# maxnorman569/Variational-Gridded-Gaussian-Processes

Hardware: NVIDIA B200
Metric: elbo_fwd_bwd_observations_per_sec (higher is better)
Workload: dtype f32

## Files before the change

### variational-gridded-gaussian-processes_b200/csrc/grid_b1.cuh

```cuda
#pragma once
#include "grid.cuh"

namespace vggp {

constexpr int FP_THREADS = 256;
constexpr int FP_WARPS = FP_THREADS / 32;
constexpr int FP_MAX_TASKS = 14;
constexpr int GEN_CHUNK = 32;
constexpr int GEN_THREADS = 256;
constexpr int FP_DET_BAND = 0;
constexpr int FP_DET_MALPHA = 3 * 512;
constexpr int FP_DET_TR = FP_DET_MALPHA + 1;
constexpr int FP_DET_LOGDET = FP_DET_TR + 8;
constexpr int FP_DET_SLOT = FP_DET_LOGDET + 8;

enum FpKind {
    FP_R = 0,
    FP_PROD,
    FP_ALPHA,
    FP_GA,
    FP_GAONLY,
    FP_DM,
    FP_DL,
    FP_QROW
};

struct FpTask {
    int kind, d, n, F;
    i64 inner, nfib;
    int tile0, ntiles;
    const double* s0;
    const double* s1;
    double* o0;
    const void* t0;
    void* t1;
    int direct;
    int pk;
};

struct FpPass {
    FpTask t[FP_MAX_TASKS];
    int ntasks;
    int D, obs_f32;
    i64 M;
    double ell_scale;
    const double* theta;
    double* gen[VGGP_MAX_D];
    double* acc[VGGP_MAX_D];
    double* sc;
    double* Qb[VGGP_MAX_D];
    void* bandT;
    int tab_off[VGGP_MAX_D];
    double* det;
    long long* dbg;
};

struct Mob { double a, b, c, d; };

__device__ __forceinline__ double pow2_inv_scale(double x) {
    const int e = (__double2hiint(x) >> 20) & 0x7ff;
    return __hiloint2double((2046 - e) << 20, 0);
}
__device__ __forceinline__ void mob_rescale(Mob& m) {
    const double sc = pow2_inv_scale(fmax(fmax(fabs(m.a), fabs(m.b)), fmax(fabs(m.c), fabs(m.d))));
    m.a *= sc; m.b *= sc; m.c *= sc; m.d *= sc;
}
__device__ __forceinline__ void mob_push(Mob& m, double p, double q) {
    const double na = fma(p, m.a, -q * m.c), nb = fma(p, m.b, -q * m.d);
    m.c = m.a; m.d = m.b; m.a = na; m.b = nb;
}

struct B1Coef { double a_in, a_bd, b; };
__device__ __forceinline__ B1Coef b1_coef(const GridDims& g, const double* theta, int d) {
    B1Coef c;
    const int n = g.n[d];
    c.a_bd = factor_entry(g, theta, d, 0, 0);
    c.a_in = factor_entry(g, theta, d, 1, 1);
    c.b = factor_entry(g, theta, d, 0, 1);
    if (n < 3) c.a_in = c.a_bd;
    return c;
}

template <typename T>
__global__ void __launch_bounds__(GEN_THREADS) k_b1_gens(const __grid_constant__ GridDims g, const double* __restrict__ theta,
                                                         double* __restrict__ acc_all, int acc_total,
                                                         double* __restrict__ theta_copy) {
    extern __shared__ double sm[];
    __shared__ double red[32];
    __shared__ double carry_d[GEN_THREADS], carry_e[GEN_THREADS];
    __shared__ Mob comp_d[GEN_THREADS / 2], comp_e[GEN_THREADS / 2];
    __shared__ int bad_flag;
    const int d = blockIdx.x;
    const int n = g.n[d];
    const int tid = threadIdx.x;
    auto G = [](int k) { return k + (k >> 5); };
    const int npad = n + (n >> 5) + 1;
    double* dd = sm;
    double* ee = dd + npad;
    double* rd = ee + npad;
    double* re = rd + npad;
    if (tid == 0) bad_flag = 0;
    if (d == 0) {
        if (tid < SC_COUNT) g.sc[tid] = 0.0;
        if (tid == 0) *g.info = 0;
        if (tid < 2 * g.D + 1) theta_copy[tid] = theta[tid];
    }
    for (int i = (int)blockIdx.x * GEN_THREADS + tid; i < acc_total; i += (int)gridDim.x * GEN_THREADS) acc_all[i] = 0.0;
    const B1Coef cf = b1_coef(g, theta, d);
    const double b2 = cf.b * cf.b;
    auto diag = [&](int k) { return (k == 0 || k == n - 1) ? cf.a_bd : cf.a_in; };
    const int nch = (n + GEN_CHUNK - 1) / GEN_CHUNK;
    const bool up = tid >= GEN_THREADS / 2;
    const int ch = up ? tid - GEN_THREADS / 2 : tid;
    if (ch < nch) {
        Mob m = {1.0, 0.0, 0.0, 1.0};
        const int k0 = ch * GEN_CHUNK, k1 = min(n, k0 + GEN_CHUNK);
        if (!up) {
            for (int k = max(k0, 1); k < k1; ++k) {
                mob_push(m, diag(k), b2);
                if ((k & 7) == 7) mob_rescale(m);
            }
            mob_rescale(m);
            comp_d[ch] = m;
        } else {
            for (int k = min(k1 - 1, n - 2); k >= k0; --k) {
                mob_push(m, diag(k), b2);
                if ((k & 7) == 0) mob_rescale(m);
            }
            mob_rescale(m);
            comp_e[ch] = m;
        }
    }
    __syncthreads();
    if (tid == 0) {
        double num = cf.a_bd, den = 1.0;
        for (int c = 0; c < nch; ++c) {
            carry_d[c] = num; carry_d[GEN_THREADS / 2 + c] = den;
            const Mob m = comp_d[c];
            const double nn = fma(m.a, num, m.b * den), dn = fma(m.c, num, m.d * den);
            const double sc = pow2_inv_scale(fmax(fabs(nn), fabs(dn)));
            num = nn * sc; den = dn * sc;
        }
    } else if (tid == 32) {
        double num = cf.a_bd, den = 1.0;
        for (int c = nch - 1; c >= 0; --c) {
            carry_e[c] = num; carry_e[GEN_THREADS / 2 + c] = den;
            const Mob m = comp_e[c];
            const double nn = fma(m.a, num, m.b * den), dn = fma(m.c, num, m.d * den);
            const double sc = pow2_inv_scale(fmax(fabs(nn), fabs(dn)));
            num = nn * sc; den = dn * sc;
        }
    }
    __syncthreads();
    if (ch < nch) {
        const int k0 = ch * GEN_CHUNK, k1 = min(n, k0 + GEN_CHUNK);
        bool bad = false;
        if (!up) {
            double prev = carry_d[ch] / carry_d[GEN_THREADS / 2 + ch];
            double r = 1.0 / prev;
            int k = k0;
            if (ch == 0) { dd[G(0)] = prev; rd[G(0)] = r; bad = !(prev > 0.0); k = 1; }
            for (; k < k1; ++k) {
                const double nxt = fma(-b2, r, diag(k));
                bad = bad || !(nxt > 0.0);
                double e = fma(-nxt, r, 1.0);
                double rn = fma(r, e, r);
                e = fma(-nxt, rn, 1.0);
                if (!(fabs(e) < 3e-16)) rn = 1.0 / nxt;
                r = rn;
                dd[G(k)] = nxt; rd[G(k)] = r;
            }
        } else {
            double nxt = carry_e[ch] / carry_e[GEN_THREADS / 2 + ch];
            double r = 1.0 / nxt;
            int k = k1 - 1;
            if (k1 == n) { ee[G(n - 1)] = nxt; re[G(n - 1)] = r; bad = !(nxt > 0.0); k = n - 2; }
            for (; k >= k0; --k) {
                const double cur = fma(-b2, r, diag(k));
                bad = bad || !(cur > 0.0);
                double e = fma(-cur, r, 1.0);
                double rn = fma(r, e, r);
                e = fma(-cur, rn, 1.0);
                if (!(fabs(e) < 3e-16)) rn = 1.0 / cur;
                r = rn;
                ee[G(k)] = cur; re[G(k)] = r;
            }
        }
        if (bad) bad_flag = 1;
    }
    __syncthreads();
    if (tid == 0 && bad_flag) atomicMax(g.info, d + 1);
    double* gen = g.gen[d];
    double prod = 1.0;
    double ld = 0.0;
    for (int i = tid; i < n; i += GEN_THREADS) {
        const double di = dd[G(i)];
        const double pdv = 1.0 / (di + ee[G(i)] - diag(i));
        const double ruv = (i + 1 < n) ? -cf.b * rd[G(i)] : 0.0;
        const double rlv = (i + 1 < n) ? -cf.b * re[G(i + 1)] : 0.0;
        gen[i] = pdv; gen[n + i] = ruv; gen[2 * n + i] = rlv;
        ee[G(i)] = pdv; dd[G(i)] = ruv;
        prod *= di;
        if (prod > 1e200 || prod < 1e-200) { ld += log(prod); prod = 1.0; }
    }
    ld += log(prod);
    __syncthreads();
    T* tab = reinterpret_cast<T*>(g.bandT) + g.tab_off[d];
    for (int i = tid; i < n; i += GEN_THREADS) {
        const bool last = (i + 1 >= n);
        const double A = ee[G(i)];
        const double B2 = last ? 0.0 : 2.0 * ee[G(i + 1)] * dd[G(i)];
        const double Cc = last ? 0.0 : ee[G(i + 1)];
        tab[i] = (T)A; tab[n + i] = (T)(B2 - 2.0 * A); tab[2 * n + i] = (T)(A - B2 + Cc);
    }
    ld = block_sum(ld, red);
    if (tid == 0) g.sc[SC_LOGDETK + d] = ld;
}

struct FpGeom {
    int n, S, pitch;
    unsigned magic;
};
__host__ __device__ inline FpGeom fp_geom(int n) {
    FpGeom q;
    q.n = n;
    q.S = (n + 31) / 32;
    int len = n + (n + q.S - 1) / q.S + 1;
    if (len < 32 * (q.S + 1) + 16) len = 32 * (q.S + 1) + 16;
    len = (len + 15) / 16 * 16 + 2;
    q.pitch = len;
    q.magic = (unsigned)((0x100000000ull + (unsigned long long)q.S - 1) / (unsigned long long)q.S);
    return q;
}
__host__ __device__ inline size_t fp_smem_bytes(int n, int F, bool aux) {
    const FpGeom q = fp_geom(n);
    const int narr = 1 + (aux ? 1 : 0) + (q.S > 16 ? 1 : 0);
    return sizeof(double) * ((size_t)5 * q.pitch + (size_t)narr * F * q.pitch);
}
__device__ __forceinline__ int fp_pidx(int i, unsigned SM) { return SM ? i + (int)__umulhi((unsigned)i, SM) : 2 * i; }

__host__ __device__ inline bool fp_kind_has_aux(int kind) { return kind == FP_GA || kind == FP_GAONLY || kind == FP_DL; }

__device__ __forceinline__ void fp_fibre(const FpGeom& q, const double* __restrict__ pd, const double* __restrict__ ru,
                                         const double* __restrict__ rl, double* __restrict__ X, double* __restrict__ U, int lane) {
    const int S = q.S, n = q.n;
    const int i0 = lane * S;
    const int cnt = max(0, min(S, n - i0));
    const int p0 = lane * (S + 1);
    double lA = 1.0, lB = 0.0, uA = 1.0, uB = 0.0;
    double sv[16];
    if (S <= 16) {
#pragma unroll
        for (int j = 0; j < 16; ++j) sv[j] = pd[p0 + j] * X[p0 + j];
#pragma unroll
        for (int j = 0; j < 16; ++j) {
            const double r = rl[p0 + j];
            const double nb = fma(r, lB, r * sv[j]), na = lA * r;
            lB = (j < cnt) ? nb : lB;
            lA = (j < cnt) ? na : lA;
        }
#pragma unroll
        for (int j = 15; j >= 0; --j) {
            const double rr = ru[j > 0 ? p0 + j - 1 : (p0 >= 2 ? p0 - 2 : 0)];
            const double r = (i0 + j > 0) ? rr : 0.0;
            const double nb = fma(r, uB, r * sv[j]), na = uA * r;
            uB = (j < cnt) ? nb : uB;
            uA = (j < cnt) ? na : uA;
        }
    } else {
        for (int j = 0; j < cnt; ++j) {
            const double r = rl[p0 + j];
            const double s = pd[p0 + j] * X[p0 + j];
            lB = fma(r, lB, r * s);
            lA *= r;
        }
        for (int j = cnt - 1; j >= 0; --j) {
            const double r = (i0 + j > 0) ? ru[j > 0 ? p0 + j - 1 : p0 - 2] : 0.0;
            const double s = pd[p0 + j] * X[p0 + j];
            uB = fma(r, uB, r * s);
            uA *= r;
        }
    }
#pragma unroll
    for (int o = 1; o < 32; o <<= 1) {
        const double Ap = __shfl_sync(0xffffffffu, lA, (lane - o) & 31), Bp = __shfl_sync(0xffffffffu, lB, (lane - o) & 31);
        const double Aq = __shfl_sync(0xffffffffu, uA, (lane + o) & 31), Bq = __shfl_sync(0xffffffffu, uB, (lane + o) & 31);
        if (lane >= o) { lB = fma(lA, Bp, lB); lA *= Ap; }
        if (lane + o < 32) { uB = fma(uA, Bq, uB); uA *= Aq; }
    }
    double l = __shfl_sync(0xffffffffu, lB, (lane - 1) & 31);
    double u = __shfl_sync(0xffffffffu, uB, (lane + 1) & 31);
    if (lane == 0) l = 0.0;
    if (lane == 31) u = 0.0;
    if (S <= 16) {
        double uu[16];
#pragma unroll
        for (int j = 15; j >= 0; --j) {
            uu[j] = u;
            const double rr = ru[j > 0 ? p0 + j - 1 : (p0 >= 2 ? p0 - 2 : 0)];
// ... 276 lines not shown
            const double* __restrict__ al = tk.s1;
            (void)al;
            for (int e = tid; e < total; e += FP_THREADS) {
                int i, f; split(e, i, f);
                if (!live(f)) continue;
                const i64 a = addr(i, f);
                const int pp = fp_pidx(i, SM);
                const double y = X[(size_t)f * q.pitch + pp];
                dst[a] = tk.direct ? y - Cx[(size_t)f * q.pitch + pp] : y;
            }
            fp_band_dots(q, X, Cx, nsrc, nsrc + nf, P.acc[d]);
        } break;
        case FP_GAONLY:
            fp_band_dots(q, X, Cx, 0, nf, P.acc[d]);
            break;
        case FP_DL: {
            double* __restrict__ dL = tk.o0;
            const double* __restrict__ L = tk.s1;
            double trO = 1.0;
            for (int e2 = 0; e2 < P.D; ++e2)
                if (e2 != d) trO *= P.sc[SC_TR + e2];
            const double ratio = (double)P.M / (double)n;
            for (int e = tid; e < total; e += FP_THREADS) {
                int i, f; split_s(e, i, f);
                if (f >= nf) continue;
                const i64 k = fib0 + f;
                const int p = fp_pidx(i, SM);
                double v = 0.0;
                if ((i64)i >= k) {
                    v = X[(size_t)f * q.pitch + p] - trO * Cx[(size_t)f * q.pitch + p];
                    if ((i64)i == k) v += ratio / L[(i64)i * n + k];
                }
                dL[(i64)i * n + k] = v;
            }
            fp_band_dots(q, X, Cx, 0, nf, P.acc[d]);
        } break;
        default: break;
    }
    __syncthreads();
    FP_STAMP(4);
#undef FP_STAMP
}

template <typename T>
__device__ __forceinline__ void fp_qrow(const FpPass& P, const FpTask& tk, int tile) {
    const int d = tk.d, n = tk.n;
    const int lane = threadIdx.x & 31;
    const int i = tile * FP_WARPS + (threadIdx.x >> 5);
    if (i >= n) return;
    const double* __restrict__ R = tk.s0;
    const double* __restrict__ L = tk.s1;
    const bool last = (i + 1 >= n);
    const double* Ri = R + (i64)i * n;
    const double* Rn = R + (i64)(last ? i : i + 1) * n;
    const double* Li = L + (i64)i * n;
    double qd = 0.0, qo = 0.0, qn = 0.0, tr = 0.0;
#pragma unroll 8
    for (int k = lane; k < n; k += 32) {
        const double r = Ri[k], rn = Rn[k];
        qd = fma(r, r, qd);
        qo = fma(r, rn, qo);
        qn = fma(rn, rn, qn);
        if (k <= i) tr = fma(r, Li[k], tr);
    }
    qd = warp_sum(qd); qo = warp_sum(qo); qn = warp_sum(qn); tr = warp_sum(tr);
    if (lane == 0) {
        if (last) { qo = 0.0; qn = 0.0; }
        P.Qb[d][i] = qd;
        P.Qb[d][n + i] = qo;
        T* tab = reinterpret_cast<T*>(P.bandT) + P.tab_off[d];
        const double B2 = 2.0 * qo;
        tab[3 * n + i] = (T)qd; tab[4 * n + i] = (T)(B2 - 2.0 * qd); tab[5 * n + i] = (T)(qd - B2 + qn);
        if (P.det) {
            double* ds = P.det + (i64)blockIdx.x * FP_DET_SLOT;
            ds[FP_DET_TR + (threadIdx.x >> 5)] = tr;
            ds[FP_DET_LOGDET + (threadIdx.x >> 5)] = 2.0 * log(fabs(Li[i]));
        } else {
            atomicAdd(P.sc + SC_TR + d, tr);
            atomicAdd(P.sc + SC_LOGDETS + d, 2.0 * log(fabs(Li[i])));
        }
    }
}

template <bool ASC, typename FA, typename FB>
__device__ __forceinline__ void warp_recurrence(int n, FA a, FB b, double* __restrict__ out, int lane) {
    const int S = (n + 31) / 32;
    const int seg = ASC ? lane : 31 - lane;
    const int i0 = seg * S, cnt = max(0, min(S, n - i0));
    const int q0 = seg * (S + 1);
    double A = 1.0, B = 0.0;
    for (int j = 0; j < cnt; ++j) {
        const int jj = ASC ? j : cnt - 1 - j;
        const double ai = a(i0 + jj, q0 + jj);
        B = fma(ai, B, b(i0 + jj, q0 + jj));
        A *= ai;
    }
#pragma unroll
    for (int o = 1; o < 32; o <<= 1) {
        const double Ap = __shfl_sync(0xffffffffu, A, (lane - o) & 31), Bp = __shfl_sync(0xffffffffu, B, (lane - o) & 31);
        if (lane >= o) { B = fma(A, Bp, B); A *= Ap; }
    }
    double t = __shfl_sync(0xffffffffu, B, (lane - 1) & 31);
    if (lane == 0) t = 0.0;
    for (int j = 0; j < cnt; ++j) {
        const int jj = ASC ? j : cnt - 1 - j;
        t = fma(a(i0 + jj, q0 + jj), t, b(i0 + jj, q0 + jj));
        out[q0 + jj] = t;
    }
}

template <typename T>
__global__ void __launch_bounds__(512) k_b1_theta(const __grid_constant__ GridDims g, const double* __restrict__ theta,
                                                  const double* __restrict__ acc, const T* __restrict__ gband,
                                                  const double* __restrict__ gscal,
                                                  double ell_scale, double* __restrict__ out, double* __restrict__ dtheta,
                                                  long long* __restrict__ dbg) {
    extern __shared__ double sm[];
    const int d = blockIdx.x;
    const int n = g.n[d];
    const int D = g.D;
    const int lane = threadIdx.x & 31, warp = threadIdx.x >> 5;
#ifndef VGGP_EMUL
#define TH_STAMP(k) do { if (dbg && threadIdx.x == 0) dbg[blockIdx.x * 8 + (k)] = clock64(); } while (0)
#else
#define TH_STAMP(k) do { } while (0)
#endif
    TH_STAMP(0);
    const int S = (n + 31) / 32;
    const int np = n + (n + S - 1) / S + 2;
    const unsigned SM = (unsigned)((0x100000000ull + (unsigned)S - 1) / (unsigned)S);
    auto P_ = [&](int i) { return fp_pidx(i, SM); };
    double* Tt = sm;
    double* Ss = sm + np;
    double* pd = sm + 2 * np;
    double* ru = sm + 3 * np;
    double* rl = sm + 4 * np;
    double* xd = sm + 5 * np;
    double* xo = sm + 6 * np;
    const double half_ratio = 0.5 * (double)g.M / (double)n;
    const double half_c = 0.5 * tr_others(g, d);
    const double cP = ell_scale / (2.0 * theta[2 * D]);
    {
        const double* __restrict__ gen = g.gen[d];
        const T* __restrict__ bp = gband + g.band_off[d];
        for (int i = threadIdx.x; i < n; i += 512) {
            const int p = P_(i);
            pd[p] = gen[i]; ru[p] = gen[n + i]; rl[p] = gen[2 * n + i];
            xd[p] = cP * (double)bp[i]; xo[p] = cP * (double)bp[n + i];
        }
    }
    for (int e = 0; e < d; ++e) acc += 3 * g.n[e];
    __syncthreads();
    TH_STAMP(1);
    if (warp == 0) {
        warp_recurrence<false>(n,
            [&](int i, int p) { return (i + 1 < n) ? ru[p] * ru[p] : 0.0; },
            [&](int i, int p) { const double x = xd[p] * pd[p] * pd[p];
                                return (i + 1 < n) ? x + 2.0 * xo[p] * pd[p] * (ru[p] * pd[P_(i + 1)]) : x; },
            Tt, lane);
    } else if (warp == 1) {
        warp_recurrence<true>(n,
            [&](int i, int p) { return (i > 0) ? rl[P_(i - 1)] * rl[P_(i - 1)] : 0.0; },
            [&](int i, int p) { const double x = xd[p] * pd[p] * pd[p];
                                if (i == 0) return x;
                                const int pm = P_(i - 1);
                                return x + 2.0 * xo[pm] * pd[p] * (rl[pm] * pd[pm]); },
            Ss, lane);
    }
    double gl[3], gs[3];
    factor_entry_grad(g, theta, d, 0, 0, gl[0], gs[0]);
    factor_entry_grad(g, theta, d, 1, 1, gl[1], gs[1]);
    factor_entry_grad(g, theta, d, 0, 1, gl[2], gs[2]);
    const double* __restrict__ Qb = g.Qb[d];
    TH_STAMP(2);
    __syncthreads();
    TH_STAMP(3);
    double sl = 0.0, ss = 0.0;
#pragma unroll 3
    for (int e = threadIdx.x; e < 3 * n; e += 512) {
        const int dl = (e >= 2 * n) ? 1 : (e >= n ? 0 : -1);
        const int i = e - (dl + 1) * n;
        const int j = i + dl;
        if (j < 0 || j >= n) continue;
        const int lo = i < j ? i : j;
        double qv, pij, w;
        if (dl == 0) {
            const int p = P_(i);
            qv = Qb[i];
            pij = pd[p];
            w = Tt[p];
            if (i > 0) {
                const int pm = P_(i - 1);
                const double pl = rl[pm] * pd[pm];
                w += rl[pm] * rl[pm] * Ss[pm] + 2.0 * xo[pm] * pl * pd[p];
            }
        } else {
            const int p = P_(lo), pn = P_(lo + 1);
            qv = Qb[n + lo];
            const double pu = ru[p] * pd[pn];
            pij = pu;
            w = ru[p] * Tt[pn] + rl[p] * Ss[p] + xo[p] * (pd[p] * pd[pn] + pu * pu);
        }
        const double v = -(acc[e] + w) + half_c * qv - half_ratio * pij;
        const bool corner = (i == 0 || i == n - 1);
        sl = fma(v, (dl != 0) ? gl[2] : (corner ? gl[0] : gl[1]), sl);
        ss = fma(v, (dl != 0) ? gs[2] : (corner ? gs[0] : gs[1]), ss);
    }
    sl = warp_sum(sl);
    ss = warp_sum(ss);
    __shared__ double red2[2][16];
    if (lane == 0) { red2[0][warp] = sl; red2[1][warp] = ss; }
    __syncthreads();
    TH_STAMP(4);
    if (threadIdx.x == 0) {
        sl = 0.0; ss = 0.0;
        for (int w = 0; w < 16; ++w) { sl += red2[0][w]; ss += red2[1][w]; }
        const double noise = theta[2 * D];
        double kff = 1.0;
        for (int e = 0; e < D; ++e) kff *= theta[D + e];
        const double E = gscal[0], nobs = gscal[1];
        const double dkff = -ell_scale * nobs / (2.0 * noise);
        dtheta[d] = sl;
        dtheta[D + d] = ss + dkff * kff / theta[D + d];
        if (d == 0) {
            const double tot = E + nobs * kff;
            const double ell = -0.5 * nobs * log(2.0 * 3.14159265358979323846 * noise) - tot / (2.0 * noise);
            dtheta[2 * D] = ell_scale * (-nobs / (2.0 * noise) + tot / (2.0 * noise * noise));
            double trp = 1.0, lds = 0.0;
            for (int e = 0; e < D; ++e) {
                trp *= g.sc[SC_TR + e];
                lds += ((double)g.M / (double)g.n[e]) * (g.sc[SC_LOGDETK + e] - g.sc[SC_LOGDETS + e]);
            }
            const double kl = 0.5 * (trp + g.sc[SC_MALPHA] - (double)g.M + lds);
            out[0] = ell_scale * ell - kl;
            out[1] = ell_scale * ell;
            out[2] = kl;
            out[3] = nobs;
        }
    }
    TH_STAMP(5);
#undef TH_STAMP
}

__global__ void __launch_bounds__(256) k_b1_fill_Kraw(const __grid_constant__ GridDims g, const double* __restrict__ theta) {
    const int d = blockIdx.y;
    const int n = g.n[d];
    const i64 e = (i64)blockIdx.x * blockDim.x + threadIdx.x;
    if (e >= (i64)n * n) return;
    g.Kraw[d][e] = factor_entry(g, theta, d, (int)(e / n), (int)(e % n));
}

}
```

### variational-gridded-gaussian-processes_b200/csrc/vggp.cu

```cuda
#include <vector>
#include <algorithm>
#include <new>
#include <mutex>

#include <cub/device/device_radix_sort.cuh>

#include "common.cuh"
#include "gemm.cuh"
#include "grid.cuh"
#include "grid_b1.cuh"
#include "grid_b1_fast.cuh"
#include "obs.cuh"
#include "obs_binned.cuh"
#include "metrics.cuh"
#include "b0scan.cuh"
#include "collective.cuh"

struct DeviceGuard {
    int prev = -1, want = -1;
    explicit DeviceGuard(int dev) : want(dev) {
        if (dev < 0 || cudaGetDevice(&prev) != cudaSuccess) { prev = -1; return; }
        if (prev != dev) cudaSetDevice(dev); else prev = -1;
    }
    ~DeviceGuard() { if (prev >= 0) cudaSetDevice(prev); }
// ... 587 lines not shown
    int pk = 0;
    while ((512 >> (pk + 1)) >= npad && (g_fp_pack == 2 || t.nfib / ((i64)nsrc << (pk + 1)) >= 296)) ++pk;
    return pk;
}

FpTask fp_mode_task(const vggp_plan* p, int kind, int e) {
    i64 outer = 1, inner = 1;
    for (int f = 0; f < e; ++f) outer *= p->n[f];
    for (int f = e + 1; f < p->D; ++f) inner *= p->n[f];
    return fp_task(p, kind, e, outer, inner);
}

void fp_pass_init(const vggp_plan* p, FpPass& P, const double* theta, double ell_scale) {
    memset(&P, 0, sizeof(P));
    P.D = p->D; P.obs_f32 = p->obs_dtype == VGGP_F32; P.M = p->M;
    P.ell_scale = ell_scale; P.theta = theta;
    int off = 0;
    for (int d = 0; d < p->D; ++d) {
        P.gen[d] = p->g.gen[d];
        P.acc[d] = p->b1_acc + off;
        off += 3 * p->n[d];
        P.Qb[d] = p->g.Qb[d];
        P.tab_off[d] = p->tab_off[d];
    }
    P.sc = p->g.sc;
    P.bandT = p->tables;
    P.dbg = g_fp_dbg;
}

int det_reserve(void** buf, size_t* have, size_t want, cudaStream_t st);
int g_fp_fast = 1;

int fp_launch(vggp_plan* p, FpPass& P, cudaStream_t st) {
    if (P.ntasks == 0) return 0;
    int tiles = 0;
    size_t smem = 0, smem_fast = 0;
    bool fast = g_fp_fast != 0;
    for (int i = 0; i < P.ntasks; ++i)
        if (P.t[i].kind != FP_QROW && (P.t[i].n > 512 || P.t[i].F != FF_F)) fast = false;
    for (int i = 0; i < P.ntasks; ++i) {
        FpTask& t = P.t[i];
        if (t.kind != FP_QROW) {
            const bool aux = fp_kind_has_aux(t.kind);
            smem = std::max(smem, fp_smem_bytes(t.n, t.F, aux));
            smem_fast = std::max(smem_fast, ff_smem_bytes(aux));
            const int nsrc = (t.kind == FP_GA) ? t.F / 2 : t.F;
            t.pk = fast ? fp_pack_log2(t) : 0;
            t.ntiles = (int)((t.nfib + ((i64)nsrc << t.pk) - 1) / ((i64)nsrc << t.pk));
        }
        t.tile0 = tiles;
        tiles += t.ntiles;
    }
    const int ti = p->obs_dtype == VGGP_F32 ? 0 : 1;
    if (p->det) {
        if (!fast) return fail(VGGP_E_UNSUPPORTED, "deterministic mode needs the fast fibre engine (M_d <= 512)");
        void* buf = p->det_fp; size_t have = p->det_fp_elems * sizeof(double);
        const int rc = det_reserve(&buf, &have, (size_t)tiles * FP_DET_SLOT * sizeof(double), st);
        p->det_fp = reinterpret_cast<double*>(buf); p->det_fp_elems = have / sizeof(double);
        if (rc) return rc;
        P.det = p->det_fp;
    }
    if (fast) {
        if (int rc = ti == 0 ? raise_dyn_smem(k_fibre_pass_fast<float>, smem_fast) : raise_dyn_smem(k_fibre_pass_fast<double>, smem_fast)) return rc;
        if (ti == 0) k_fibre_pass_fast<float><<<tiles, FP_THREADS, smem_fast, st>>>(P);
        else k_fibre_pass_fast<double><<<tiles, FP_THREADS, smem_fast, st>>>(P);
        VGGP_LAUNCH_CHECK();
        if (P.det) {
            k_fp_det_reduce<<<dim3(P.D, FP_DET_YB), 256, 0, st>>>(P);
            VGGP_LAUNCH_CHECK();
        }
        return 0;
    }
    if (int rc = ti == 0 ? raise_dyn_smem(k_fibre_pass<float>, smem) : raise_dyn_smem(k_fibre_pass<double>, smem)) return rc;
    if (ti == 0) k_fibre_pass<float><<<tiles, FP_THREADS, smem, st>>>(P);
    else k_fibre_pass<double><<<tiles, FP_THREADS, smem, st>>>(P);
    VGGP_LAUNCH_CHECK();
    return 0;
}

int b1f_forward(vggp_plan* p, const double* theta, const double* m, const double* L, cudaStream_t st) {
    const int D = p->D;
    int rc;
    const size_t gsm = 4 * ((size_t)p->nmax + p->nmax / 32 + 1) * sizeof(double);
    if (p->obs_dtype == VGGP_F32) k_b1_gens<float><<<D, GEN_THREADS, gsm, st>>>(p->g, theta, p->b1_acc, p->b1_acc_total, p->theta_dev);
    else k_b1_gens<double><<<D, GEN_THREADS, gsm, st>>>(p->g, theta, p->b1_acc, p->b1_acc_total, p->theta_dev);
    VGGP_LAUNCH_CHECK();
    FpPass P;
    auto qrows = [&](FpPass& Q) {
        for (int d = 0; d < D; ++d) {
            FpTask t = fp_task(p, FP_QROW, d, 1, p->n[d]);
            t.s0 = p->g.R[d]; t.s1 = L + p->g.Loff[d];
            Q.t[Q.ntasks++] = t;
        }
    };
    fp_pass_init(p, P, theta, 1.0);
    for (int d = 0; d < D; ++d) {
        FpTask t = fp_task(p, FP_R, d, 1, p->n[d]);
        t.s0 = L + p->g.Loff[d]; t.o0 = p->g.R[d];
        P.t[P.ntasks++] = t;
    }
    {
        FpTask t = fp_mode_task(p, D == 1 ? FP_ALPHA : FP_PROD, 0);
        t.s0 = m; t.s1 = m;
        t.o0 = D == 1 ? p->alpha : p->pgA;
        t.t1 = p->alphaT;
        P.t[P.ntasks++] = t;
    }
    if ((rc = fp_launch(p, P, st))) return rc;
    const double* src = p->pgA;
    if (D == 3) {
        fp_pass_init(p, P, theta, 1.0);
        FpTask t = fp_mode_task(p, FP_PROD, 1);
        t.s0 = p->pgA; t.o0 = p->pgB;
        P.t[P.ntasks++] = t;
        qrows(P);
        if ((rc = fp_launch(p, P, st))) return rc;
        src = p->pgB;
    }
    fp_pass_init(p, P, theta, 1.0);
    if (D >= 2) {
        FpTask t = fp_mode_task(p, FP_ALPHA, D - 1);
        t.s0 = src; t.s1 = m; t.o0 = p->alpha; t.t1 = p->alphaT;
        P.t[P.ntasks++] = t;
    }
    if (D != 3) qrows(P);
    return fp_launch(p, P, st);
}

int b1f_backward(vggp_plan* p, const double* theta, const double* m, const double* L, const void* gbuf, double ell_scale,
                 double* out, double* dtheta, double* dm, double* dL, cudaStream_t st) {
    const int D = p->D;
    int rc;
    const size_t tsz = p->obs_dtype == VGGP_F32 ? 4 : 8;
    i64 n_elems, soff, nsc, total;
    vggp_gbuf_layout(p, &n_elems, &soff, &nsc, &total);
    const unsigned char* gb = reinterpret_cast<const unsigned char*>(gbuf);
    const double* gscal = reinterpret_cast<const double*>(gb + soff);
    auto band = [&](int d) { return (const void*)(gb + ((size_t)p->M + p->band_off[d]) * tsz); };
    FpPass P;
    fp_pass_init(p, P, theta, ell_scale);
    {
        FpTask t = fp_mode_task(p, FP_GA, D - 1);
        t.s0 = m; t.s1 = p->alpha; t.t0 = gbuf;
        t.direct = (D == 1);
        t.o0 = D == 1 ? dm : p->pgA;
        P.t[P.ntasks++] = t;
    }
    if ((rc = fp_launch(p, P, st))) return rc;
    fp_pass_init(p, P, theta, ell_scale);
    if (D >= 2) {
        const int e = D - 2;
        FpTask t = fp_mode_task(p, e == 0 ? FP_DM : FP_PROD, e);
        t.s0 = p->pgA; t.s1 = p->alpha; t.o0 = e == 0 ? dm : p->pgB;
        P.t[P.ntasks++] = t;
        FpTask a = fp_mode_task(p, FP_GAONLY, e);
        a.s0 = m; a.s1 = p->alpha; a.t0 = gbuf;
        P.t[P.ntasks++] = a;
    }
    for (int d = 0; d < D; ++d) {
        FpTask t = fp_task(p, FP_DL, d, 1, p->n[d]);
        t.s0 = p->g.R[d]; t.s1 = L + p->g.Loff[d]; t.t0 = band(d); t.o0 = dL + p->g.Loff[d];
        P.t[P.ntasks++] = t;
    }
    if ((rc = fp_launch(p, P, st))) return rc;
    if (D == 3) {
        fp_pass_init(p, P, theta, ell_scale);
        FpTask t = fp_mode_task(p, FP_DM, 0);
        t.s0 = p->pgB; t.s1 = p->alpha; t.o0 = dm;
// ... 1955 lines not shown
```

Before: 341.1 billion.

## Cache recurrence operands in registers and prefetch theta-kernel global loads early

The warp recurrence now keeps up to 16 a/b operand pairs per lane in registers, so the second pass reuses them instead of recomputing them from shared memory. The theta kernel issues its acc/Qb global loads before the first barrier, which lets them overlap the serial recurrences. It also moves the scalar ELBO/KL output computation onto an idle warp during the recurrence instead of after the final reduction. This adds register pressure under a 512-thread launch bound and only applies the register path when the segment length is at most 16.

```diff
diff --git a/variational-gridded-gaussian-processes_b200/csrc/grid_b1.cuh b/variational-gridded-gaussian-processes_b200/csrc/grid_b1.cuh
--- a/variational-gridded-gaussian-processes_b200/csrc/grid_b1.cuh
+++ b/variational-gridded-gaussian-processes_b200/csrc/grid_b1.cuh
@@ -663,12 +663,31 @@
     const int seg = ASC ? lane : 31 - lane;
     const int i0 = seg * S, cnt = max(0, min(S, n - i0));
     const int q0 = seg * (S + 1);
+    constexpr int R = 16;
+    double av[R], bv[R];
+    const bool reg = S <= R;
+    if (reg) {
+#pragma unroll
+        for (int j = 0; j < R; ++j) {
+            const int jj = ASC ? j : cnt - 1 - j;
+            if (j < cnt) { av[j] = a(i0 + jj, q0 + jj); bv[j] = b(i0 + jj, q0 + jj); }
+        }
+    }
     double A = 1.0, B = 0.0;
-    for (int j = 0; j < cnt; ++j) {
-        const int jj = ASC ? j : cnt - 1 - j;
-        const double ai = a(i0 + jj, q0 + jj);
-        B = fma(ai, B, b(i0 + jj, q0 + jj));
-        A *= ai;
+    if (reg) {
+#pragma unroll
+        for (int j = 0; j < R; ++j) {
+            if (j >= cnt) break;
+            B = fma(av[j], B, bv[j]);
+            A *= av[j];
+        }
+    } else {
+        for (int j = 0; j < cnt; ++j) {
+            const int jj = ASC ? j : cnt - 1 - j;
+            const double ai = a(i0 + jj, q0 + jj);
+            B = fma(ai, B, b(i0 + jj, q0 + jj));
+            A *= ai;
+        }
     }
 #pragma unroll
     for (int o = 1; o < 32; o <<= 1) {
@@ -677,10 +696,20 @@
     }
     double t = __shfl_sync(0xffffffffu, B, (lane - 1) & 31);
     if (lane == 0) t = 0.0;
-    for (int j = 0; j < cnt; ++j) {
-        const int jj = ASC ? j : cnt - 1 - j;
-        t = fma(a(i0 + jj, q0 + jj), t, b(i0 + jj, q0 + jj));
-        out[q0 + jj] = t;
+    if (reg) {
+#pragma unroll
+        for (int j = 0; j < R; ++j) {
+            if (j >= cnt) break;
+            const int jj = ASC ? j : cnt - 1 - j;
+            t = fma(av[j], t, bv[j]);
+            out[q0 + jj] = t;
+        }
+    } else {
+        for (int j = 0; j < cnt; ++j) {
+            const int jj = ASC ? j : cnt - 1 - j;
+            t = fma(a(i0 + jj, q0 + jj), t, b(i0 + jj, q0 + jj));
+            out[q0 + jj] = t;
+        }
     }
 }
 
@@ -715,6 +744,23 @@
     const double half_ratio = 0.5 * (double)g.M / (double)n;
     const double half_c = 0.5 * tr_others(g, d);
     const double cP = ell_scale / (2.0 * theta[2 * D]);
+    for (int e = 0; e < d; ++e) acc += 3 * g.n[e];
+    constexpr int THB = 3;
+    const double* __restrict__ Qb = g.Qb[d];
+    double accv[THB], qvv[THB];
+#pragma unroll
+    for (int k = 0; k < THB; ++k) {
+        const int e = threadIdx.x + k * 512;
+        const int dl = (e >= 2 * n) ? 1 : (e >= n ? 0 : -1);
+        const int i = e - (dl + 1) * n, j = i + dl;
+        const bool ok = e < 3 * n && j >= 0 && j < n;
+        accv[k] = ok ? acc[e] : 0.0;
+        qvv[k] = ok ? Qb[dl == 0 ? i : n + (i < j ? i : j)] : 0.0;
+    }
+    double kff = 1.0;
+    for (int e = 0; e < D; ++e) kff *= theta[D + e];
+    const double noise = theta[2 * D];
+    const double nobs = gscal[1];
     {
         const double* __restrict__ gen = g.gen[d];
         const T* __restrict__ bp = gband + g.band_off[d];
@@ -724,7 +770,6 @@
             xd[p] = cP * (double)bp[i]; xo[p] = cP * (double)bp[n + i];
         }
     }
-    for (int e = 0; e < d; ++e) acc += 3 * g.n[e];
     __syncthreads();
     TH_STAMP(1);
     if (warp == 0) {
@@ -741,27 +786,39 @@
                                 const int pm = P_(i - 1);
                                 return x + 2.0 * xo[pm] * pd[p] * (rl[pm] * pd[pm]); },
             Ss, lane);
+    } else if (warp == 2 && lane == 0 && d == 0) {
+        const double E = gscal[0];
+        const double tot = E + nobs * kff;
+        const double ell = -0.5 * nobs * log(2.0 * 3.14159265358979323846 * noise) - tot / (2.0 * noise);
+        dtheta[2 * D] = ell_scale * (-nobs / (2.0 * noise) + tot / (2.0 * noise * noise));
+        double trp = 1.0, lds = 0.0;
+        for (int e = 0; e < D; ++e) {
+            trp *= g.sc[SC_TR + e];
+            lds += ((double)g.M / (double)g.n[e]) * (g.sc[SC_LOGDETK + e] - g.sc[SC_LOGDETS + e]);
+        }
+        const double kl = 0.5 * (trp + g.sc[SC_MALPHA] - (double)g.M + lds);
+        out[0] = ell_scale * ell - kl;
+        out[1] = ell_scale * ell;
+        out[2] = kl;
+        out[3] = nobs;
     }
     double gl[3], gs[3];
     factor_entry_grad(g, theta, d, 0, 0, gl[0], gs[0]);
     factor_entry_grad(g, theta, d, 1, 1, gl[1], gs[1]);
     factor_entry_grad(g, theta, d, 0, 1, gl[2], gs[2]);
-    const double* __restrict__ Qb = g.Qb[d];
     TH_STAMP(2);
     __syncthreads();
     TH_STAMP(3);
     double sl = 0.0, ss = 0.0;
-#pragma unroll 3
-    for (int e = threadIdx.x; e < 3 * n; e += 512) {
+    auto term = [&](int e, double acc_e, double qv) {
         const int dl = (e >= 2 * n) ? 1 : (e >= n ? 0 : -1);
         const int i = e - (dl + 1) * n;
         const int j = i + dl;
-        if (j < 0 || j >= n) continue;
+        if (j < 0 || j >= n) return;
         const int lo = i < j ? i : j;
-        double qv, pij, w;
+        double pij, w;
         if (dl == 0) {
             const int p = P_(i);
-            qv = Qb[i];
             pij = pd[p];
             w = Tt[p];
             if (i > 0) {
@@ -771,15 +828,24 @@
             }
         } else {
             const int p = P_(lo), pn = P_(lo + 1);
-            qv = Qb[n + lo];
             const double pu = ru[p] * pd[pn];
             pij = pu;
             w = ru[p] * Tt[pn] + rl[p] * Ss[p] + xo[p] * (pd[p] * pd[pn] + pu * pu);
         }
-        const double v = -(acc[e] + w) + half_c * qv - half_ratio * pij;
+        const double v = -(acc_e + w) + half_c * qv - half_ratio * pij;
         const bool corner = (i == 0 || i == n - 1);
         sl = fma(v, (dl != 0) ? gl[2] : (corner ? gl[0] : gl[1]), sl);
         ss = fma(v, (dl != 0) ? gs[2] : (corner ? gs[0] : gs[1]), ss);
+    };
+#pragma unroll
+    for (int k = 0; k < THB; ++k) {
+        const int e = threadIdx.x + k * 512;
+        if (e < 3 * n) term(e, accv[k], qvv[k]);
+    }
+    for (int e = threadIdx.x + THB * 512; e < 3 * n; e += 512) {
+        const int dl = (e >= 2 * n) ? 1 : (e >= n ? 0 : -1);
+        const int i = e - (dl + 1) * n, j = i + dl;
+        if (j >= 0 && j < n) term(e, acc[e], Qb[dl == 0 ? i : n + (i < j ? i : j)]);
     }
     sl = warp_sum(sl);
     ss = warp_sum(ss);
@@ -790,28 +856,9 @@
     if (threadIdx.x == 0) {
         sl = 0.0; ss = 0.0;
         for (int w = 0; w < 16; ++w) { sl += red2[0][w]; ss += red2[1][w]; }
-        const double noise = theta[2 * D];
-        double kff = 1.0;
-        for (int e = 0; e < D; ++e) kff *= theta[D + e];
-        const double E = gscal[0], nobs = gscal[1];
         const double dkff = -ell_scale * nobs / (2.0 * noise);
         dtheta[d] = sl;
         dtheta[D + d] = ss + dkff * kff / theta[D + d];
-        if (d == 0) {
-            const double tot = E + nobs * kff;
-            const double ell = -0.5 * nobs * log(2.0 * 3.14159265358979323846 * noise) - tot / (2.0 * noise);
-            dtheta[2 * D] = ell_scale * (-nobs / (2.0 * noise) + tot / (2.0 * noise * noise));
-            double trp = 1.0, lds = 0.0;
-            for (int e = 0; e < D; ++e) {
-                trp *= g.sc[SC_TR + e];
-                lds += ((double)g.M / (double)g.n[e]) * (g.sc[SC_LOGDETK + e] - g.sc[SC_LOGDETS + e]);
-            }
-            const double kl = 0.5 * (trp + g.sc[SC_MALPHA] - (double)g.M + lds);
-            out[0] = ell_scale * ell - kl;
-            out[1] = ell_scale * ell;
-            out[2] = kl;
-            out[3] = nobs;
-        }
     }
     TH_STAMP(5);
 #undef TH_STAMP
```

Result: faster. 345.8 billion, median of 6 (+1.4%).

## Parallelize band-gradient recurrences across full block and prefetch band operands

Applied to the files above, without the earlier changes.

The two backward recurrences in the band-gradient kernel were each run by a single warp. They now use a 256-thread block-level scan per direction, with register-held segments and a cross-warp carry through shared memory. Band accumulator and Qb loads, theta and scalar reads, and the factor gradients are hoisted ahead of the first barrier so their latency overlaps the recurrences. The ELBO output is computed by a separate thread instead of the final reducer. The generator kernel's Möbius rescale is folded into the push, clock64 timing stamps are added, and the kernel's dynamic shared memory limit is raised explicitly. The block scan caps elements per thread at BR_MAXE, which limits the supported n.

```diff
diff --git a/variational-gridded-gaussian-processes_b200/csrc/grid_b1.cuh b/variational-gridded-gaussian-processes_b200/csrc/grid_b1.cuh
--- a/variational-gridded-gaussian-processes_b200/csrc/grid_b1.cuh
+++ b/variational-gridded-gaussian-processes_b200/csrc/grid_b1.cuh
@@ -8,6 +8,7 @@
 constexpr int FP_MAX_TASKS = 14;
 constexpr int GEN_CHUNK = 32;
 constexpr int GEN_THREADS = 256;
+constexpr int GEN_DBG_ROW = 4088;
 constexpr int FP_DET_BAND = 0;
 constexpr int FP_DET_MALPHA = 3 * 512;
 constexpr int FP_DET_TR = FP_DET_MALPHA + 1;
@@ -70,6 +71,12 @@
     m.c = m.a; m.d = m.b; m.a = na; m.b = nb;
 }
 
+__device__ __forceinline__ void mob_push_rescaled(Mob& m, double p, double q) {
+    const double sc = pow2_inv_scale(fmax(fmax(fabs(m.a), fabs(m.b)), fmax(fabs(m.c), fabs(m.d))));
+    const double na = fma(p, m.a, -q * m.c), nb = fma(p, m.b, -q * m.d);
+    m.c = m.a * sc; m.d = m.b * sc; m.a = na * sc; m.b = nb * sc;
+}
+
 struct B1Coef { double a_in, a_bd, b; };
 __device__ __forceinline__ B1Coef b1_coef(const GridDims& g, const double* theta, int d) {
     B1Coef c;
@@ -84,7 +91,7 @@
 template <typename T>
 __global__ void __launch_bounds__(GEN_THREADS) k_b1_gens(const __grid_constant__ GridDims g, const double* __restrict__ theta,
                                                          double* __restrict__ acc_all, int acc_total,
-                                                         double* __restrict__ theta_copy) {
+                                                         double* __restrict__ theta_copy, long long* __restrict__ dbg) {
     extern __shared__ double sm[];
     __shared__ double red[32];
     __shared__ double carry_d[GEN_THREADS], carry_e[GEN_THREADS];
@@ -93,6 +100,12 @@
     const int d = blockIdx.x;
     const int n = g.n[d];
     const int tid = threadIdx.x;
+#ifndef VGGP_EMUL
+#define GEN_STAMP(k) do { if (dbg && tid == 0) dbg[(GEN_DBG_ROW + d) * 8 + (k)] = clock64(); } while (0)
+#else
+#define GEN_STAMP(k) do { } while (0)
+#endif
+    GEN_STAMP(0);
     auto G = [](int k) { return k + (k >> 5); };
     const int npad = n + (n >> 5) + 1;
     double* dd = sm;
@@ -117,28 +130,29 @@
         const int k0 = ch * GEN_CHUNK, k1 = min(n, k0 + GEN_CHUNK);
         if (!up) {
             for (int k = max(k0, 1); k < k1; ++k) {
-                mob_push(m, diag(k), b2);
-                if ((k & 7) == 7) mob_rescale(m);
+                if ((k & 7) == 7) mob_push_rescaled(m, diag(k), b2);
+                else mob_push(m, diag(k), b2);
             }
             mob_rescale(m);
             comp_d[ch] = m;
         } else {
             for (int k = min(k1 - 1, n - 2); k >= k0; --k) {
-                mob_push(m, diag(k), b2);
-                if ((k & 7) == 0) mob_rescale(m);
+                if ((k & 7) == 0) mob_push_rescaled(m, diag(k), b2);
+                else mob_push(m, diag(k), b2);
             }
             mob_rescale(m);
             comp_e[ch] = m;
         }
     }
     __syncthreads();
+    GEN_STAMP(1);
     if (tid == 0) {
         double num = cf.a_bd, den = 1.0;
         for (int c = 0; c < nch; ++c) {
             carry_d[c] = num; carry_d[GEN_THREADS / 2 + c] = den;
             const Mob m = comp_d[c];
+            const double sc = pow2_inv_scale(fmax(fabs(num), fabs(den)));
             const double nn = fma(m.a, num, m.b * den), dn = fma(m.c, num, m.d * den);
-            const double sc = pow2_inv_scale(fmax(fabs(nn), fabs(dn)));
             num = nn * sc; den = dn * sc;
         }
     } else if (tid == 32) {
@@ -146,12 +160,13 @@
         for (int c = nch - 1; c >= 0; --c) {
             carry_e[c] = num; carry_e[GEN_THREADS / 2 + c] = den;
             const Mob m = comp_e[c];
+            const double sc = pow2_inv_scale(fmax(fabs(num), fabs(den)));
             const double nn = fma(m.a, num, m.b * den), dn = fma(m.c, num, m.d * den);
-            const double sc = pow2_inv_scale(fmax(fabs(nn), fabs(dn)));
             num = nn * sc; den = dn * sc;
         }
     }
     __syncthreads();
+    GEN_STAMP(2);
     if (ch < nch) {
         const int k0 = ch * GEN_CHUNK, k1 = min(n, k0 + GEN_CHUNK);
         bool bad = false;
@@ -189,6 +204,7 @@
         if (bad) bad_flag = 1;
     }
     __syncthreads();
+    GEN_STAMP(3);
     if (tid == 0 && bad_flag) atomicMax(g.info, d + 1);
     double* gen = g.gen[d];
     double prod = 1.0;
@@ -215,6 +231,8 @@
     }
     ld = block_sum(ld, red);
     if (tid == 0) g.sc[SC_LOGDETK + d] = ld;
+    GEN_STAMP(4);
+#undef GEN_STAMP
 }
 
 struct FpGeom {
@@ -657,31 +675,37 @@
     }
 }
 
-template <bool ASC, typename FA, typename FB>
-__device__ __forceinline__ void warp_recurrence(int n, FA a, FB b, double* __restrict__ out, int lane) {
-    const int S = (n + 31) / 32;
-    const int seg = ASC ? lane : 31 - lane;
-    const int i0 = seg * S, cnt = max(0, min(S, n - i0));
-    const int q0 = seg * (S + 1);
+constexpr int BR_MAXE = 10;
+template <int NT, typename FAB, typename FOUT>
+__device__ __forceinline__ void block_recurrence(int n, int r, bool asc, FAB ab, FOUT out, double* __restrict__ wsc) {
+    constexpr int NW = NT / 32;
+    const int lane = r & 31, w = r >> 5;
+    const int S = (n + NT - 1) / NT;
+    const int s0 = r * S, cnt = max(0, min(S, n - s0));
+    double a[BR_MAXE], b[BR_MAXE];
     double A = 1.0, B = 0.0;
-    for (int j = 0; j < cnt; ++j) {
-        const int jj = ASC ? j : cnt - 1 - j;
-        const double ai = a(i0 + jj, q0 + jj);
-        B = fma(ai, B, b(i0 + jj, q0 + jj));
-        A *= ai;
-    }
+#pragma unroll
+    for (int j = 0; j < BR_MAXE; ++j)
+        if (j < cnt) ab(asc ? s0 + j : n - 1 - s0 - j, a[j], b[j]);
+#pragma unroll
+    for (int j = 0; j < BR_MAXE; ++j)
+        if (j < cnt) { B = fma(a[j], B, b[j]); A *= a[j]; }
 #pragma unroll
     for (int o = 1; o < 32; o <<= 1) {
         const double Ap = __shfl_sync(0xffffffffu, A, (lane - o) & 31), Bp = __shfl_sync(0xffffffffu, B, (lane - o) & 31);
         if (lane >= o) { B = fma(A, Bp, B); A *= Ap; }
     }
-    double t = __shfl_sync(0xffffffffu, B, (lane - 1) & 31);
-    if (lane == 0) t = 0.0;
-    for (int j = 0; j < cnt; ++j) {
-        const int jj = ASC ? j : cnt - 1 - j;
-        t = fma(a(i0 + jj, q0 + jj), t, b(i0 + jj, q0 + jj));
-        out[q0 + jj] = t;
-    }
+    if (lane == 31) { wsc[w] = A; wsc[NW + w] = B; }
+    const double Al = __shfl_sync(0xffffffffu, A, (lane - 1) & 31), Bl = __shfl_sync(0xffffffffu, B, (lane - 1) & 31);
+    __syncthreads();
+    double t = 0.0;
+#pragma unroll
+    for (int v = 0; v < NW - 1; ++v)
+        if (v < w) t = fma(wsc[v], t, wsc[NW + v]);
+    if (lane > 0) t = fma(Al, t, Bl);
+#pragma unroll
+    for (int j = 0; j < BR_MAXE; ++j)
+        if (j < cnt) { t = fma(a[j], t, b[j]); out(asc ? s0 + j : n - 1 - s0 - j, t); }
 }
 
 template <typename T>
@@ -715,6 +739,37 @@
     const double half_ratio = 0.5 * (double)g.M / (double)n;
     const double half_c = 0.5 * tr_others(g, d);
     const double cP = ell_scale / (2.0 * theta[2 * D]);
+    for (int e = 0; e < d; ++e) acc += 3 * g.n[e];
+    const double* __restrict__ Qb = g.Qb[d];
+    constexpr int BAND_PF = 3;
+    double pf_acc[BAND_PF], pf_q[BAND_PF];
+#pragma unroll
+    for (int u = 0; u < BAND_PF; ++u) {
+        const int e = threadIdx.x + u * 512;
+        const int dl = (e >= 2 * n) ? 1 : (e >= n ? 0 : -1);
+        const int i = e - (dl + 1) * n, j = i + dl;
+        const bool ok = e < 3 * n && j >= 0 && j < n;
+        pf_acc[u] = ok ? acc[e] : 0.0;
+        pf_q[u] = ok ? Qb[dl == 0 ? i : n + min(i, j)] : 0.0;
+    }
+    const bool elbo_thread = (d == 0 && threadIdx.x == 32);
+    double t_noise = 1.0, t_kff = 1.0, t_E = 0.0, t_nobs = 0.0, t_s2 = 1.0, t_trp = 1.0, t_lds = 0.0, t_ma = 0.0;
+    if (threadIdx.x == 0 || elbo_thread) {
+        t_noise = theta[2 * D];
+        for (int e = 0; e < D; ++e) t_kff *= theta[D + e];
+        t_E = gscal[0]; t_nobs = gscal[1]; t_s2 = theta[D + d];
+        if (elbo_thread) {
+            for (int e = 0; e < D; ++e) {
+                t_trp *= g.sc[SC_TR + e];
+                t_lds += ((double)g.M / (double)g.n[e]) * (g.sc[SC_LOGDETK + e] - g.sc[SC_LOGDETS + e]);
+            }
+            t_ma = g.sc[SC_MALPHA];
+        }
+    }
+    double gl[3], gs[3];
+    factor_entry_grad(g, theta, d, 0, 0, gl[0], gs[0]);
+    factor_entry_grad(g, theta, d, 1, 1, gl[1], gs[1]);
+    factor_entry_grad(g, theta, d, 0, 1, gl[2], gs[2]);
     {
         const double* __restrict__ gen = g.gen[d];
         const T* __restrict__ bp = gband + g.band_off[d];
@@ -724,44 +779,41 @@
             xd[p] = cP * (double)bp[i]; xo[p] = cP * (double)bp[n + i];
         }
     }
-    for (int e = 0; e < d; ++e) acc += 3 * g.n[e];
     __syncthreads();
     TH_STAMP(1);
-    if (warp == 0) {
-        warp_recurrence<false>(n,
-            [&](int i, int p) { return (i + 1 < n) ? ru[p] * ru[p] : 0.0; },
-            [&](int i, int p) { const double x = xd[p] * pd[p] * pd[p];
-                                return (i + 1 < n) ? x + 2.0 * xo[p] * pd[p] * (ru[p] * pd[P_(i + 1)]) : x; },
-            Tt, lane);
-    } else if (warp == 1) {
-        warp_recurrence<true>(n,
-            [&](int i, int p) { return (i > 0) ? rl[P_(i - 1)] * rl[P_(i - 1)] : 0.0; },
-            [&](int i, int p) { const double x = xd[p] * pd[p] * pd[p];
-                                if (i == 0) return x;
-                                const int pm = P_(i - 1);
-                                return x + 2.0 * xo[pm] * pd[p] * (rl[pm] * pd[pm]); },
-            Ss, lane);
-    }
-    double gl[3], gs[3];
-    factor_entry_grad(g, theta, d, 0, 0, gl[0], gs[0]);
-    factor_entry_grad(g, theta, d, 1, 1, gl[1], gs[1]);
-    factor_entry_grad(g, theta, d, 0, 1, gl[2], gs[2]);
-    const double* __restrict__ Qb = g.Qb[d];
+    {
+        __shared__ double wsc[2][16];
+        const int grp = threadIdx.x >> 8;
+        block_recurrence<256>(n, threadIdx.x & 255, grp == 1,
+            [&](int i, double& a, double& b) {
+                const int p = P_(i);
+                const double x = xd[p] * pd[p] * pd[p];
+                if (grp == 0) {
+                    a = (i + 1 < n) ? ru[p] * ru[p] : 0.0;
+                    b = (i + 1 < n) ? x + 2.0 * xo[p] * pd[p] * (ru[p] * pd[P_(i + 1)]) : x;
+                } else if (i == 0) {
+                    a = 0.0; b = x;
+                } else {
+                    const int pm = P_(i - 1);
+                    a = rl[pm] * rl[pm];
+                    b = x + 2.0 * xo[pm] * pd[p] * (rl[pm] * pd[pm]);
+                }
+            },
+            [&](int i, double t) { (grp == 0 ? Tt : Ss)[P_(i)] = t; }, wsc[grp]);
+    }
     TH_STAMP(2);
     __syncthreads();
     TH_STAMP(3);
     double sl = 0.0, ss = 0.0;
-#pragma unroll 3
-    for (int e = threadIdx.x; e < 3 * n; e += 512) {
+    auto band_term = [&](int e, double accv, double qv) {
         const int dl = (e >= 2 * n) ? 1 : (e >= n ? 0 : -1);
         const int i = e - (dl + 1) * n;
         const int j = i + dl;
-        if (j < 0 || j >= n) continue;
+        if (j < 0 || j >= n) return;
         const int lo = i < j ? i : j;
-        double qv, pij, w;
+        double pij, w;
         if (dl == 0) {
             const int p = P_(i);
-            qv = Qb[i];
             pij = pd[p];
             w = Tt[p];
             if (i > 0) {
@@ -771,47 +823,48 @@
             }
         } else {
             const int p = P_(lo), pn = P_(lo + 1);
-            qv = Qb[n + lo];
             const double pu = ru[p] * pd[pn];
             pij = pu;
             w = ru[p] * Tt[pn] + rl[p] * Ss[p] + xo[p] * (pd[p] * pd[pn] + pu * pu);
         }
-        const double v = -(acc[e] + w) + half_c * qv - half_ratio * pij;
+        const double v = -(accv + w) + half_c * qv - half_ratio * pij;
         const bool corner = (i == 0 || i == n - 1);
         sl = fma(v, (dl != 0) ? gl[2] : (corner ? gl[0] : gl[1]), sl);
         ss = fma(v, (dl != 0) ? gs[2] : (corner ? gs[0] : gs[1]), ss);
+    };
+#pragma unroll
+    for (int u = 0; u < BAND_PF; ++u) {
+        const int e = threadIdx.x + u * 512;
+        if (e < 3 * n) band_term(e, pf_acc[u], pf_q[u]);
+    }
+    for (int e = threadIdx.x + BAND_PF * 512; e < 3 * n; e += 512) {
+        const int dl = (e >= 2 * n) ? 1 : (e >= n ? 0 : -1);
+        const int i = e - (dl + 1) * n, j = i + dl;
+        if (j < 0 || j >= n) continue;
+        band_term(e, acc[e], Qb[dl == 0 ? i : n + min(i, j)]);
     }
     sl = warp_sum(sl);
     ss = warp_sum(ss);
     __shared__ double red2[2][16];
     if (lane == 0) { red2[0][warp] = sl; red2[1][warp] = ss; }
+    if (elbo_thread) {
+        const double tot = t_E + t_nobs * t_kff;
+        const double ell = -0.5 * t_nobs * log(2.0 * 3.14159265358979323846 * t_noise) - tot / (2.0 * t_noise);
+        dtheta[2 * D] = ell_scale * (-t_nobs / (2.0 * t_noise) + tot / (2.0 * t_noise * t_noise));
+        const double kl = 0.5 * (t_trp + t_ma - (double)g.M + t_lds);
+        out[0] = ell_scale * ell - kl;
+        out[1] = ell_scale * ell;
+        out[2] = kl;
+        out[3] = t_nobs;
+    }
     __syncthreads();
     TH_STAMP(4);
     if (threadIdx.x == 0) {
         sl = 0.0; ss = 0.0;
         for (int w = 0; w < 16; ++w) { sl += red2[0][w]; ss += red2[1][w]; }
-        const double noise = theta[2 * D];
-        double kff = 1.0;
-        for (int e = 0; e < D; ++e) kff *= theta[D + e];
-        const double E = gscal[0], nobs = gscal[1];
-        const double dkff = -ell_scale * nobs / (2.0 * noise);
+        const double dkff = -ell_scale * t_nobs / (2.0 * t_noise);
         dtheta[d] = sl;
-        dtheta[D + d] = ss + dkff * kff / theta[D + d];
-        if (d == 0) {
-            const double tot = E + nobs * kff;
-            const double ell = -0.5 * nobs * log(2.0 * 3.14159265358979323846 * noise) - tot / (2.0 * noise);
-            dtheta[2 * D] = ell_scale * (-nobs / (2.0 * noise) + tot / (2.0 * noise * noise));
-            double trp = 1.0, lds = 0.0;
-            for (int e = 0; e < D; ++e) {
-                trp *= g.sc[SC_TR + e];
-                lds += ((double)g.M / (double)g.n[e]) * (g.sc[SC_LOGDETK + e] - g.sc[SC_LOGDETS + e]);
-            }
-            const double kl = 0.5 * (trp + g.sc[SC_MALPHA] - (double)g.M + lds);
-            out[0] = ell_scale * ell - kl;
-            out[1] = ell_scale * ell;
-            out[2] = kl;
-            out[3] = nobs;
-        }
+        dtheta[D + d] = ss + dkff * t_kff / t_s2;
     }
     TH_STAMP(5);
 #undef TH_STAMP
diff --git a/variational-gridded-gaussian-processes_b200/csrc/vggp.cu b/variational-gridded-gaussian-processes_b200/csrc/vggp.cu
--- a/variational-gridded-gaussian-processes_b200/csrc/vggp.cu
+++ b/variational-gridded-gaussian-processes_b200/csrc/vggp.cu
@@ -693,8 +693,9 @@
     const int D = p->D;
     int rc;
     const size_t gsm = 4 * ((size_t)p->nmax + p->nmax / 32 + 1) * sizeof(double);
-    if (p->obs_dtype == VGGP_F32) k_b1_gens<float><<<D, GEN_THREADS, gsm, st>>>(p->g, theta, p->b1_acc, p->b1_acc_total, p->theta_dev);
-    else k_b1_gens<double><<<D, GEN_THREADS, gsm, st>>>(p->g, theta, p->b1_acc, p->b1_acc_total, p->theta_dev);
+    if (int rc = p->obs_dtype == VGGP_F32 ? raise_dyn_smem(k_b1_gens<float>, gsm) : raise_dyn_smem(k_b1_gens<double>, gsm)) return rc;
+    if (p->obs_dtype == VGGP_F32) k_b1_gens<float><<<D, GEN_THREADS, gsm, st>>>(p->g, theta, p->b1_acc, p->b1_acc_total, p->theta_dev, g_fp_dbg);
+    else k_b1_gens<double><<<D, GEN_THREADS, gsm, st>>>(p->g, theta, p->b1_acc, p->b1_acc_total, p->theta_dev, g_fp_dbg);
     VGGP_LAUNCH_CHECK();
     FpPass P;
     auto qrows = [&](FpPass& Q) {
```

After: 341.8 billion before, 346.7 billion after, median of 6. 1.4% higher.
